# alitteneker/jsraytracer

Measured on AMD Instinct MI355X. Metric: pixel-samples/sec + %HBM-roofline, cornell_box_path 1024² @1/2/4/8 GPU, higher is better.
Workload: dtype f64; 1 GPU; cornell_box_path 1024x1024 64spp depth 8 (Incremental); width=1024, height=1024, spp=64, max_depth=8, parallelism=tiles1, col_block=1, headline=True, gather=rgba8

## Files before the change

jsraytracer_amd/csrc/device_common.h:

```cpp
#pragma once
#include <hip/hip_runtime.h>
#include <stdint.h>

#include "device_scene.h"
#include "fdlibm.h"
#include "js_number.h"

#define JSRT_HD __host__ __device__ __forceinline__

namespace jsrt {

#define JS_PI 3.141592653589793
#define DINF __builtin_inf()

JSRT_HD bool is_nan(double x) { return x != x; }
JSRT_HD double js_max(double a, double b) {
    double r = a > b ? a : b;
    if (a == b) r = __builtin_bit_cast(double, __builtin_bit_cast(uint64_t, a) & __builtin_bit_cast(uint64_t, b));
    return a != a ? a : r;
}
JSRT_HD double js_min(double a, double b) {
    double r = a < b ? a : b;
    if (a == b) r = __builtin_bit_cast(double, __builtin_bit_cast(uint64_t, a) | __builtin_bit_cast(uint64_t, b));
    return a != a ? a : r;
// ... 819 lines not shown
    }
    return res;
}

struct Hit {
    double t;
    int prim;
    int ctx;
};

template <int PF, class PT>
__device__ __forceinline__ double prim_intersect_local(const DScene &S, const PT &P, F3 o, F3 d, double minD,
                                                       double maxD) {
    switch (P.gkind) {
    case JSRT_GEOM_PLANE: return plane_t(o, d);
    case JSRT_GEOM_SQUARE: {
        const double t = plane_t(o, d);
        const F3 p = ray_point(o, d, t);
        return (-0.5f <= p.x && p.x <= 0.5f && -0.5f <= p.y && p.y <= 0.5f) ? t : -DINF;
    }
    case JSRT_GEOM_CIRCLE: {
        const double t = plane_t(o, d);
        const F3 p = ray_point(o, d, t);
        return (dot3(p, p) <= 1) ? t : -DINF;
    }
    case JSRT_GEOM_SPHERE: return sphere_static(o, d, minD);
    case JSRT_GEOM_CYLINDER: {
        const double oz = o.z, dz = d.z;
        if (fabs(oz) > 1 && dz != 0) minD = js_max(minD, -(oz - js_sign(oz)) / dz);
        const double t = sphere_static(f3(o.x, o.y, o.z * 0.0f), f3(d.x, d.y, d.z * 0.0f), minD);
        return (fabs(oz + t * dz) <= 1) ? t : -DINF;
    }
    case JSRT_GEOM_AABB: return aabb_intersect(P.center, P.half, o, d, minD, maxD);
    case JSRT_GEOM_TRIANGLE:
        if (PF & PF_TRI) return tri_intersect(S.tris[P.gindex], o, d);
        return -DINF;
    case JSRT_GEOM_SDF:
        if (PF & PF_SDF) return sdf_intersect(S, P.gindex, o, d, minD, maxD);
        return -DINF;
    default: return -DINF;
    }
}

template <class T>
JSRT_HD float xf_row_point(const T *r, F3 o) {
    return (float)((((double)o.x * r[0] + (double)o.y * r[1]) + (double)o.z * r[2]) + r[3]);
}
template <class T>
JSRT_HD float xf_row_dir(const T *r, F3 d) {
    return (float)(((double)d.x * r[0] + (double)d.y * r[1]) + (double)d.z * r[2]);
}

template <class T>
JSRT_HD double planar_intersect(int k, const T *inv, F3 o, F3 d, double minD, double lim) {
    const float oz = xf_row_point(inv + 8, o), dz = xf_row_dir(inv + 8, d);
    const double t = (dz != 0.0f) ? -(double)oz / (double)dz : -(double)__builtin_inf();
    if (k == JSRT_GEOM_PLANE || !(t > minD && t < lim)) return t;
    const float ox = xf_row_point(inv, o), oy = xf_row_point(inv + 4, o);
    const float dx = xf_row_dir(inv, d), dy = xf_row_dir(inv + 4, d);
    const F3 p = ray_point(f3(ox, oy, oz), f3(dx, dy, dz), t);
    if (k == JSRT_GEOM_SQUARE)
        return (-0.5f <= p.x && p.x <= 0.5f && -0.5f <= p.y && p.y <= 0.5f) ? t : -(double)__builtin_inf();
    return (dot3(p, p) <= 1) ? t : -(double)__builtin_inf();
}

#ifdef JSRT_X_F32XF
template <class T>
__device__ __forceinline__ float xf_row_point_x(const T *r, F3 o) {
    return fmaf(o.x, (float)r[0], fmaf(o.y, (float)r[1], fmaf(o.z, (float)r[2], (float)r[3])));
}
template <class T>
__device__ __forceinline__ float xf_row_dir_x(const T *r, F3 d) {
    return fmaf(d.x, (float)r[0], fmaf(d.y, (float)r[1], d.z * (float)r[2]));
}
#define XROWP xf_row_point_x
#define XROWD xf_row_dir_x
#else
#define XROWP xf_row_point
#define XROWD xf_row_dir
#endif

template <class T>
JSRT_HD int planar_any_f32(int k, const T *inv, F3 o, F3 d, double minD, double maxD, double &t_out) {
    constexpr float EPS = 4.76837158203125e-7f, EPSP = 3.814697265625e-6f, TINY = 1e-30f;
    const float oz = XROWP(inv + 8, o), dz = XROWD(inv + 8, d);
    if (dz == 0.0f) return 0;
#ifdef __HIP_DEVICE_COMPILE__
    const float ta = -oz * __builtin_amdgcn_rcpf(dz);
#else
    const float ta = -oz * (1.0f / dz);
#endif
    const float f0 = (float)minD, f1 = (float)maxD;
    if (!__builtin_isfinite(ta) || !__builtin_isfinite(f0) || !(fabsf(dz) >= 1e-30f)) return -1;
    const bool inf1 = !__builtin_isfinite(f1) && f1 > 0;
    const float et = EPS * fabsf(ta) + TINY, e0 = EPS * fabsf(f0) + TINY, e1 = inf1 ? 0.0f : EPS * fabsf(f1) + TINY;
    if (ta + et < f0 - e0 || (!inf1 && ta - et > f1 + e1)) return 0;
    if (!(ta - et > f0 + e0 && (inf1 || ta + et < f1 - e1))) return -1;
    if (k == JSRT_GEOM_PLANE) {
        t_out = ta;
        return 1;
    }
    const float ox = XROWP(inv, o), oy = XROWP(inv + 4, o);
    const float dx = XROWD(inv, d), dy = XROWD(inv + 4, d);
    const double td = (double)ta;
    const float sx = (float)((double)dx * td), sy = (float)((double)dy * td);
    const float px = ox + sx, py = oy + sy;
    const float ex = EPSP * (fabsf(sx) + fabsf(ox)) + TINY, ey = EPSP * (fabsf(sy) + fabsf(oy)) + TINY;
    if (!__builtin_isfinite(px) || !__builtin_isfinite(py) || !__builtin_isfinite(ex) || !__builtin_isfinite(ey))
        return -1;
    if (k == JSRT_GEOM_SQUARE) {
        if (fabsf(px) - ex > 0.5f || fabsf(py) - ey > 0.5f) return 0;
        if (fabsf(px) + ex < 0.5f && fabsf(py) + ey < 0.5f) {
            t_out = ta;
            return 1;
        }
        return -1;
    }
    const float sz = (float)((double)dz * td), pz = oz + sz;
    const float ez = EPSP * (fabsf(sz) + fabsf(oz)) + TINY;
    const double r2 = dot3(f3(px, py, pz), f3(px, py, pz));
    const double m = 2.0 * ((double)fabsf(px) * ex + (double)fabsf(py) * ey + (double)fabsf(pz) * ez) +
                     ((double)ex * ex + (double)ey * ey + (double)ez * ez) + 1e-15;
    if (!__builtin_isfinite(r2)) return -1;
    if (r2 - m > 1.0) return 0;
    if (r2 + m < 1.0) {
        t_out = ta;
        return 1;
    }
    return -1;
}

JSRT_HD int sphere_any_f32(F3 o, F3 d, double minD, double maxD, double &t_out, bool *second = nullptr) {
    constexpr float EPS = 4.76837158203125e-7f, EPSS = 1.9073486328125e-6f, TINY = 1e-30f;
    const double a = dot3(d, d), b = dot3(d, o), c = dot3(o, o) - 1;
    const double big = b * b - a * c;
    if (big < 0 || a == 0) return 0;
    if (!(big >= 1e-30) || !(a >= 1e-30) || !(a <= 1e30) || !(fabs(b) <= 1e30) || !(big <= 1e30)) return -1;
    const float fa = (float)a, fb = (float)b;
#ifdef __HIP_DEVICE_COMPILE__
    const float sq = __builtin_amdgcn_sqrtf((float)big), ia = __builtin_amdgcn_rcpf(fa);
#else
    const float sq = sqrtf((float)big), ia = 1.0f / fa;
#endif
    const float t1 = (-fb + sq) * ia, t2 = (-fb - sq) * ia;
    const float base = EPSS * (sq * ia);
    const float e1 = base + EPSS * fabsf(t1) + TINY, e2 = base + EPSS * fabsf(t2) + TINY;
    const float f0 = (float)minD, f1 = (float)maxD;
    if (!__builtin_isfinite(f0)) return -1;
    const bool inf1 = !__builtin_isfinite(f1) && f1 > 0;
    const float em = EPS * fabsf(f0) + TINY, eM = inf1 ? 0.0f : EPS * fabsf(f1) + TINY;
    float t, et;
    if (t2 - e2 > f0 + em) {
        t = t2;
        et = e2;
        if (second) *second = true;
// ... 17 lines not shown
    bool second = false;
    const int dec = sphere_any_f32(o, d, minD, lim, te, &second);
    if (dec != 1) return dec;
    const double a = dot3(d, d), b = dot3(d, o), c = dot3(o, o) - 1;
    const double big = sqrt(b * b - a * c);
    t_out = second ? (-b - big) / a : (-b + big) / a;
    return 1;
}

template <int PF, class PT>
__device__ __forceinline__ double prim_intersect(const DScene &S, const PT &P, F3 o, F3 d, double minD, double maxD,
                                                 bool transp, double lim) {
    if (!transp && !P.casts_shadow) return DINF;
    const int k = P.gkind;
    if (k == JSRT_GEOM_PLANE || k == JSRT_GEOM_SQUARE || k == JSRT_GEOM_CIRCLE) return planar_intersect(k, P.inv, o, d, minD, lim);
    return prim_intersect_local<PF>(S, P, xf_point(P.inv, o), xf_dir(P.inv, d), minD, maxD);
}

template <int PF, class PT>
__device__ __forceinline__ double prim_any(const DScene &S, const PT &P, F3 o, F3 d, double minD, double maxD,
                                           bool transp) {
#ifndef JSRT_NO_ANY_FILTER
    if (!transp && !P.casts_shadow) return DINF;
    const int k = P.gkind;
    double t = 0;
    if (k == JSRT_GEOM_AABB) {
#ifdef JSRT_X_F32XF
        const F3 lo = f3(XROWP(P.inv, o), XROWP(P.inv + 4, o), XROWP(P.inv + 8, o)),
                 ld = f3(XROWD(P.inv, d), XROWD(P.inv + 4, d), XROWD(P.inv + 8, d));
#else
        const F3 lo = xf_point(P.inv, o), ld = xf_dir(P.inv, d);
#endif
        const int dec = box_any_f32(P.center, P.half, lo, box_ray(ld), minD, maxD, t);
        if (dec >= 0) return dec ? t : -DINF;
        return aabb_intersect(P.center, P.half, lo, ld, minD, maxD);
    }
    if (k == JSRT_GEOM_PLANE || k == JSRT_GEOM_SQUARE || k == JSRT_GEOM_CIRCLE) {
        const int dec = planar_any_f32(k, P.inv, o, d, minD, maxD, t);
        if (dec >= 0) return dec ? t : -DINF;
        return planar_intersect(k, P.inv, o, d, minD, maxD);
    }
    if ((PF & PF_TRI) && k == JSRT_GEOM_TRIANGLE)
        return tri_any(S.tris[P.gindex], xf_point(P.inv, o), xf_dir(P.inv, d), minD, maxD);
    if (k == JSRT_GEOM_SPHERE) {
        const F3 lo = xf_point(P.inv, o), ld = xf_dir(P.inv, d);
        const int dec = sphere_any_f32(lo, ld, minD, maxD, t);
        if (dec >= 0) return dec ? t : -DINF;
        return sphere_static(lo, ld, minD);
    }
#endif
    return prim_intersect<PF>(S, P, o, d, minD, maxD, transp, maxD);
}

template <int PF, class PT>
__device__ __forceinline__ double prim_closest(const DScene &S, const PT &P, F3 o, F3 d, double minD, double maxD,
                                               bool transp, double lim) {
#if !defined(JSRT_NO_ANY_FILTER) && !defined(JSRT_NO_CLOSEST_FILTER)
    if constexpr (!(PF & PF_BVH)) {
        if (!transp && !P.casts_shadow) return DINF;
        const int k = P.gkind;
        double t = 0;
        if (k == JSRT_GEOM_AABB) {
            const F3 lo = xf_point(P.inv, o), ld = xf_dir(P.inv, d);
            const int dec = box_closest_f32(P.center, P.half, lo, ld, box_ray(ld), minD, lim, t);
            if (dec >= 0) return dec ? t : -DINF;
            return aabb_intersect(P.center, P.half, lo, ld, minD, maxD);
        }
        if (k == JSRT_GEOM_SPHERE) {
            const F3 lo = xf_point(P.inv, o), ld = xf_dir(P.inv, d);
            const int dec = sphere_closest_f32(lo, ld, minD, lim, t);
            if (dec >= 0) return dec ? t : -DINF;
            return sphere_static(lo, ld, minD);
        }
    }
#endif
    return prim_intersect<PF>(S, P, o, d, minD, maxD, transp, lim);
}

template <int PF, bool ANY>
__device__ __forceinline__ Hit bvh_cast(const DScene &S, const DInst &I, F3 o, F3 d, double minD, double maxD, bool transp) {
    Hit best{DINF, -1, I.ctx};
    const bool fast = I.count != 0;
    extern __shared__ int bvh_lds_stack[];
    int *const stack = bvh_lds_stack + threadIdx.x;
    const int stride = (int)blockDim.x;
    const BoxRay br = box_ray(d);
    const float fmin_d = (float)minD;
    float flim = (float)maxD;
    int sp = 0;
    stack[0] = I.first;
    ++sp;
    while (sp > 0) {
        --sp;
        const DBvhNode N = S.bvh[stack[sp * stride]];
#ifndef JSRT_NO_BOX_FILTER
        int en = box_enter_f32(N.cx, N.cy, N.cz, N.hx, N.hy, N.hz, o, br, fmin_d, flim);
#else
        int en = -1;
#endif
        if (en < 0) {
            double tmn, tmx;
            en = aabb_slab(N.cx, N.cy, N.cz, N.hx, N.hy, N.hz, o, d, minD, maxD, tmn, tmx) && tmn <= maxD &&
                 tmx >= minD && tmn <= best.t;
        }
        if (en) {
            if (N.b < 0) {
// ... 14 lines not shown
            } else {
                stack[sp * stride] = N.a;
                stack[(sp + 1) * stride] = N.b;
                sp += 2;
            }
        }
    }
    return best;
}

template <int PF, bool ANY>
__device__ __forceinline__ void nested_cast(const DScene &S, int inst, F3 o, F3 d, double minD, double maxD, bool transp, Hit &best) {
    struct Fr {
        int inst, next;
        F3 o, d;
    };
    Fr st[8];
    int sp = 0;
    {
        const DInst &I = S.insts[inst];
        st[sp++] = Fr{inst, 0, xf_point(S.mats + 12 * I.matrix, o), xf_dir(S.mats + 12 * I.matrix, d)};
    }
    while (sp > 0) {
        Fr &f = st[sp - 1];
        const DInst &I = S.insts[f.inst];
        if (I.kind == INST_BVH) {
            const Hit h = bvh_cast<PF, ANY>(S, I, f.o, f.d, minD, maxD, transp);
            --sp;
            if (h.prim >= 0 && h.t > minD && h.t < best.t && h.t < maxD) {
                best = h;
                if (ANY) return;
            }
            continue;
        }
        if (f.next >= I.count) { --sp; continue; }
        const int c = S.inst_child[I.first + f.next++];
        const DInst &C = S.insts[c];
        if (C.kind == INST_PRIM) {
            const double t = ANY ? prim_any<PF>(S, S.prims[C.prim], f.o, f.d, minD, maxD, transp)
                                 : prim_intersect<PF>(S, S.prims[C.prim], f.o, f.d, minD, maxD, transp, fmin(maxD, best.t));
            if (t > minD && t < best.t && t < maxD) {
                best = Hit{t, C.prim, I.ctx};
                if (ANY) return;
            }
        } else if (sp < 8) {
            const double *m = S.mats + 12 * C.matrix;
            const F3 no = xf_point(m, f.o), nd = xf_dir(m, f.d);
            st[sp++] = Fr{c, 0, no, nd};
        }
    }
}

template <class RBT>
__device__ __forceinline__ bool root_needed(const RBT &RB, F3 o, float ix, float iy, float iz, float oabs,
                                            float fminD, float flim) {
    if (!RB.bounded) return true;
    const float e = RB.k * oabs + RB.e0;
    float a0 = (RB.lo[0] - e - o.x) * ix, a1 = (RB.hi[0] + e - o.x) * ix;
    float tn = fminf(a0, a1), tf = fmaxf(a0, a1);
    a0 = (RB.lo[1] - e - o.y) * iy;
    a1 = (RB.hi[1] + e - o.y) * iy;
    tn = fmaxf(tn, fminf(a0, a1));
    tf = fminf(tf, fmaxf(a0, a1));
    a0 = (RB.lo[2] - e - o.z) * iz;
    a1 = (RB.hi[2] + e - o.z) * iz;
    tn = fmaxf(tn, fminf(a0, a1));
    tf = fminf(tf, fmaxf(a0, a1));
    return (tn <= tf) && (tf >= fminD) && (tn <= flim);
}

template <int PF, bool ANY>
__device__ __forceinline__ Hit world_cast(const DScene &S, F3 o, F3 d, double minD, double maxD, bool transp,
                                          uint64_t mask = ~0ull) {
    Hit best{DINF, -1, 0};
    const float ix = __builtin_amdgcn_rcpf(d.x), iy = __builtin_amdgcn_rcpf(d.y), iz = __builtin_amdgcn_rcpf(d.z);
    const float oabs = fmaxf(fabsf(o.x), fmaxf(fabsf(o.y), fabsf(o.z)));
    const float fminD = (float)minD;
    bool live = true;
    float flim = (float)maxD;
    for (int i = 0; i < S.n_roots; ++i) {
        if (i < 64 && !((mask >> i) & 1ull)) continue;
        const auto &R = as_const(S.rootrec)[i];
        const bool need = live && root_needed(R.rb, o, ix, iy, iz, oabs, fminD, flim);
        if (!__any(need)) continue;
#ifdef JSRT_X_CULLONLY
        if (ANY) continue;
#endif
        if (!need) {
        } else if (R.kind == INST_PRIM) {
            if (transp || R.p.casts_shadow) {
                const double t = ANY ? prim_any<PF>(S, R.p, o, d, minD, maxD, transp)
                                     : prim_closest<PF>(S, R.p, o, d, minD, maxD, transp, fmin(maxD, best.t));
                if (t > minD && t < best.t && t < maxD) {
                    best = Hit{t, R.prim, 0};
                    flim = (float)best.t;
                    if (ANY) live = false;
                }
            }
        } else if ((PF & PF_BVH) && R.kind == INST_BVH) {
            const auto *m = R.p.inv;
            const Hit h = bvh_cast<PF, ANY>(S, S.insts[R.inst], xf_point(m, o), xf_dir(m, d), minD, maxD, transp);
            if (h.prim >= 0 && h.t > minD && h.t < best.t && h.t < maxD) {
                best = h;
                flim = (float)best.t;
                if (ANY) live = false;
            }
        } else if (PF & PF_AGG) {
            nested_cast<PF, ANY>(S, R.inst, o, d, minD, maxD, transp, best);
            flim = (float)(best.t < maxD ? best.t : maxD);
            if (ANY && best.prim >= 0) live = false;
        }
    }
    return best;
}

template <int C>
__device__ __forceinline__ bool sroot_class(const DScene &S, uint64_t m, F3 o, F3 d, double minD, double maxD,
                                            float ix, float iy, float iz, float oabs, bool &live) {
    typedef uint32_t u16v __attribute__((ext_vector_type(16)));
    typedef uint32_t u8v __attribute__((ext_vector_type(8)));
    const float fminD = (float)minD, flim = (float)maxD;
    while (m) {
        if (!__any(live)) break;
        const int j = __builtin_ctzll(m);
        m &= m - 1;
        const CONST_AS uint32_t *w = reinterpret_cast<const CONST_AS uint32_t *>(as_const(S.sroot) + j);
        u16v a = *reinterpret_cast<const CONST_AS u16v *>(w);
        u16v b = *reinterpret_cast<const CONST_AS u16v *>(w + 16);
        u8v c = *reinterpret_cast<const CONST_AS u8v *>(w + 32);
        __asm__ volatile("" : "+s"(a), "+s"(b), "+s"(c));
        double inv[12];
#pragma unroll
        for (int k = 0; k < 8; ++k) inv[k] = __hiloint2double((int)a[2 * k + 1], (int)a[2 * k]);
#pragma unroll
        for (int k = 0; k < 4; ++k) inv[8 + k] = __hiloint2double((int)b[2 * k + 1], (int)b[2 * k]);
        RootBound rb;
        rb.lo[0] = __uint_as_float(b[8]);
        rb.lo[1] = __uint_as_float(b[9]);
        rb.lo[2] = __uint_as_float(b[10]);
        rb.k = __uint_as_float(b[11]);
        rb.hi[0] = __uint_as_float(b[12]);
        rb.hi[1] = __uint_as_float(b[13]);
        rb.hi[2] = __uint_as_float(b[14]);
        rb.e0 = __uint_as_float(b[15]);
        rb.bounded = (int32_t)c[7];
        const bool need = live && root_needed(rb, o, ix, iy, iz, oabs, fminD, flim);
        if (!__any(need)) continue;
        if (!need) continue;
        double t = 0;
        if constexpr (C == SR_BOX) {
            const float ce[3] = {__uint_as_float(c[0]), __uint_as_float(c[1]), __uint_as_float(c[2])};
            const float ha[3] = {__uint_as_float(c[4]), __uint_as_float(c[5]), __uint_as_float(c[6])};
            const F3 lo = xf_point(inv, o), ld = xf_dir(inv, d);
            const int dec = box_any_f32(ce, ha, lo, box_ray(ld), minD, maxD, t);
            if (dec < 0) t = aabb_intersect(ce, ha, lo, ld, minD, maxD);
            else if (!dec) t = -DINF;
        } else if constexpr (C == SR_PLANE || C == SR_SQUARE || C == SR_CIRCLE) {
            const int k = C == SR_PLANE ? JSRT_GEOM_PLANE : C == SR_SQUARE ? JSRT_GEOM_SQUARE : JSRT_GEOM_CIRCLE;
            const int dec = planar_any_f32(k, inv, o, d, minD, maxD, t);
            if (dec < 0) t = planar_intersect(k, inv, o, d, minD, maxD);
            else if (!dec) t = -DINF;
        } else if constexpr (C == SR_SPHERE) {
            const F3 lo = xf_point(inv, o), ld = xf_dir(inv, d);
            const int dec = sphere_any_f32(lo, ld, minD, maxD, t);
            if (dec < 0) t = sphere_static(lo, ld, minD);
            else if (!dec) t = -DINF;
// ... 338 lines not shown
```

jsraytracer_amd/csrc/render.hip:

```cpp
#include "render_levels.h"

#include <mutex>

namespace jsrt {

const char *const KT_NAMES[KT_N] = {"k_gen", "k_extend", "k_shade", "k_shadow", "k_reduce", "k_accum", "k_final",
                                    "k_resolve"};

__global__ __launch_bounds__(256) void k_gen(DScene S, RenderArgs A, WArgs W) {
    const uint32_t q = blockIdx.x * 256 + threadIdx.x;
    if ((!W.chain || W.hybrid) && q < LVL_UNDER) W.lvl[q] = q == 0 ? W.npaths : 0u;
    if (q >= W.npaths) return;
    int c = 0, py = 0, px = 0;
    const uint32_t nsb = W.npaths / W.npix;
    const uint32_t pl = W.pixel_major ? q / nsb : q % W.npix, sl = W.pixel_major ? q % nsb : q / W.npix;
    const uint32_t smp = W.s0 + sl;
    const bool valid = pixel_of(A, W.p0 + pl, c, py, px);
    if (!W.chain) {
        if (A.max_depth <= 0) {
            W.root[3 * q] = W.root[3 * q + 1] = W.root[3 * q + 2] = 0.0f;
            return;
        }
        W.path[q] = q;
        W.parent[q] = valid ? NO_PARENT : DEAD_RAY;
// ... 546 lines not shown
            release_events();
            return e;
        }
    }
    hipStream_t st2 = dual ? wf.side : st;
    const char *se = getenv("JSRT_SPLIT");
    const bool split = !timed_launches && ns > 0 && (se ? se[0] == '1' : (persist && !dual));
    auto aux_of = [&](Wavefront &w) -> hipError_t {
        hipError_t r = hipSuccess;
        if (!w.aux) r = hipStreamCreateWithFlags(&w.aux, hipStreamNonBlocking);
        if (r == hipSuccess && !w.ev_shade) r = hipEventCreateWithFlags(&w.ev_shade, hipEventDisableTiming);
        if (r == hipSuccess && !w.ev_shadow) r = hipEventCreateWithFlags(&w.ev_shadow, hipEventDisableTiming);
        return r;
    };
    if (split && (e = aux_of(wf)) == hipSuccess && dual) e = aux_of(*wf.twin);
    if (e != hipSuccess) {
        if (h_lvl) (void)hipHostFree(h_lvl);
        release_events();
        return e;
    }
    bool conservative = false, aborted = false;
    double reported = 0;
    for (int attempt = 0; e == hipSuccess; ++attempt) {
        if (kt) kt->attempts = (uint32_t)attempt + 1;
        const size_t cap = hybrid ? ((paths + paths * wf.pool_factor / 4 + 255) & ~(size_t)255) : paths;
        if (hybrid && cap * (size_t)depth >= ((size_t)1 << 32)) { e = hipErrorOutOfMemory; break; }
        const size_t pool = chain ? cap : paths * wf.pool_factor, level_cap = chain ? cap : pool / 2;
        int group = 1;
        const char *ss = getenv("JSRT_SHADOW_SERIAL");
        if (ns > 1 && ns <= 64 && !(ss && ss[0] == '1' && !persist))
            while (group < ns) group *= 2;
        const size_t hands = chain ? cap : std::max(level_cap, paths);
        const size_t shadow = persist ? hands * (size_t)group : 0;
        auto reserve = [&](Wavefront &w) {
            return chain ? w.reserve(cap, cap * (size_t)depth, cap, paths, sched, shadow)
                         : w.reserve(pool, pool, hands, paths, SCHED_TREE, shadow);
        };
        e = reserve(wf);
        if (e == hipSuccess && dual) {
            const hipError_t e2 = reserve(*wf.twin);
            if (e2 == hipErrorOutOfMemory) {
                (void)hipGetLastError();
                wf.twin->release();
                dual = false;
                st2 = st;
            } else {
                e = e2;
            }
        }
        if (e != hipSuccess) break;
        WArgs W = wf.args;
        W.ns = ns;
        W.group = group;
        W.chain = chain ? 1 : 0;
        W.hybrid = hybrid ? 1 : 0;
        W.cap = (uint32_t)cap;
        const char *be = getenv("JSRT_BUCKET");
        int shift = 0;
        while (S.n_prims > 0 && ((S.n_prims - 1) >> shift) >= BKT_N) ++shift;
        W.bucket = (learned && !persist && S.n_prims > 0 && ns > 0 && ns <= 64 && !(be && be[0] == '0')) ? shift + 1 : 0;
        W.pool = pool;
        W.level_cap = level_cap;
        const char *cs = getenv("JSRT_CHILD_SORT");
        W.child_sort = !chain && (cs ? (cs[0] == '1') : ((S.profile & PF_BVH) != 0));
        const char *bg = getenv("JSRT_BUCKET_GRID");
        const bool grid = bg ? bg[0] == '1' : S.profile == PF_ANALYTIC;
        W.bucket_grid = (W.bucket && S.grid_cells > 0 && grid) ? 1 : 0;
        W.pixel_major = pixel_major ? 1 : 0;
        WArgs W2 = W;
        if (dual) {
            const WArgs &t = wf.twin->args;
            W2.ox = t.ox; W2.oy = t.oy; W2.oz = t.oz; W2.dx = t.dx; W2.dy = t.dy; W2.dz = t.dz;
            W2.addr = t.addr; W2.key = t.key; W2.path = t.path; W2.parent = t.parent; W2.t = t.t;
            W2.prim = t.prim; W2.ctx = t.ctx; W2.node = t.node; W2.child = t.child; W2.slot = t.slot;
            W2.hand = t.hand; W2.hnode = t.hnode; W2.root = t.root; W2.lvl = t.lvl; W2.qctr = t.qctr; W2.sray = t.sray;
            W2.scol = t.scol; W2.bkt = t.bkt; W2.bbase = t.bbase; W2.brank = t.brank;
            W2.list0 = t.list0; W2.list1 = t.list1; W2.endl = t.endl;
            W2.fixrec = t.fixrec; W2.fixctr = t.fixctr; W2.fixcap = t.fixcap;
        }
        if ((e = hipMemsetAsync(A.accum, 0, (size_t)A.ncols * A.H * 4 * sizeof(float), st)) != hipSuccess) break;
        if ((e = hipMemsetAsync(W.lvl + LVL_UNDER, 0, 2 * sizeof(uint32_t), st)) != hipSuccess) break;
        if ((e = hipMemsetAsync(W.fixctr, 0, sizeof(uint32_t), st)) != hipSuccess) break;
        if (dual && (e = hipMemsetAsync(W2.fixctr, 0, sizeof(uint32_t), st)) != hipSuccess) break;
        if (dual) {
            if ((e = hipEventRecord(ev_start, st)) != hipSuccess || (e = hipStreamWaitEvent(st2, ev_start, 0)) != hipSuccess) break;
            if ((e = hipMemsetAsync(W2.lvl + LVL_UNDER, 0, 2 * sizeof(uint32_t), st2)) != hipSuccess) break;
        }
        auto read_flags = [&]() -> hipError_t {
            hipError_t r;
            if (dual && ((r = hipEventRecord(ev_end, st2)) != hipSuccess || (r = hipStreamWaitEvent(st, ev_end, 0)) != hipSuccess))
                return r;
            if ((r = hipMemcpyAsync(h_lvl, W.lvl, 64 * sizeof(uint32_t), hipMemcpyDeviceToHost, st)) != hipSuccess) return r;
            if (dual && (r = hipMemcpyAsync(h_lvl + 64, W2.lvl, 64 * sizeof(uint32_t), hipMemcpyDeviceToHost, st)) != hipSuccess)
                return r;
            return hipStreamSynchronize(st);
        };
        auto flagged = [&](int k) { return h_lvl[k] != 0 || (dual && h_lvl[64 + k] != 0); };
        uint64_t bi = 0;
        auto bounds = [&](uint32_t np) {
            std::vector<size_t> b(depth, 0);
            if (hybrid) {
                for (int L = 0; L < A.max_depth; ++L) {
                    b[L] = L == 0 ? np : cap;
                    if (L > 0 && !conservative && L < (int)wf.frac.size())
                        b[L] = std::min(cap, std::max<size_t>(256, (size_t)((double)np * wf.frac[L] * margin) + slack));
                }
// ... 141 lines not shown
```

jsraytracer_amd/csrc/render_kernel.h:

```cpp
#pragma once
#include <hip/hip_runtime.h>
#include <stdint.h>

#include <functional>
#include <vector>

#include "device_scene.h"

namespace jsrt {

constexpr int MAX_TREE_DEPTH = 16;
constexpr int LVL_FLAG = 63;
constexpr int LVL_UNDER = 62;
static_assert(2 * MAX_TREE_DEPTH + 2 <= LVL_UNDER, "hybrid chain count pairs lvl[2L, 2L + 1] below the flags");
constexpr int BKT_N = 64;
constexpr int BKT_S = 16;
constexpr int BKT_K = BKT_N * BKT_S;
constexpr int BKT_LEVEL = 3 * BKT_K + 64;

struct RenderArgs {
    int32_t W, H, kind, max_depth;
    int32_t s_begin, s_end, spp;
    uint32_t seed;
    int32_t x_offset, x_delt, col_block, ncols;
    float *accum;
    uint32_t *rgba;
    float *colors;
    int32_t final_pass;
    int32_t patches_x;
    int32_t patches;
    int32_t samples_per_batch;
    int32_t tile_p;
};

constexpr uint32_t INFO_HIT = 1u, INFO_LIT = 2u, INFO_MISS = 16u;
constexpr uint32_t INFO_UNIT0 = 32u, INFO_UNIT1 = 64u;
constexpr int INFO_NCHILD_SHIFT = 2;

struct WArgs {
    float *ox, *oy, *oz, *dx, *dy, *dz;
    uint32_t *addr;
    uint32_t *key;
    uint32_t *path;
    uint32_t *parent;
    double *t;
    int32_t *prim, *ctx;
    float4 *node;
    float4 *child;
    float4 *slot;
    float4 *hand;
    uint32_t *hnode;
    float *root;
    uint32_t *lvl;
    uint32_t *list0, *list1;
    uint8_t *endl;
    uint32_t *qctr;
    uint4 *fixrec;
    uint32_t *fixctr;
    uint32_t fixcap;
    int32_t force_fix;
    float4 *sray;
    float4 *scol;
    uint32_t *bkt;
    uint32_t *bbase;
    uint32_t *brank;
    uint32_t p0, npix, s0, npaths;
    int32_t ns;
    int32_t group;
    int32_t chain;
    int32_t hybrid;
    uint32_t cap;
    int32_t bucket;
    int32_t child_sort;
    int32_t bucket_grid;
    int32_t pixel_major;
    size_t pool, level_cap;
    size_t nstride, hstride;
    size_t sstride;
};

struct BatchSync {
    hipEvent_t wait = nullptr, done = nullptr;
    hipStream_t aux = nullptr;
    hipEvent_t shade_done = nullptr, shadow_done = nullptr;
};

struct Wavefront {
    void *mem = nullptr;
    Wavefront *twin = nullptr;
    hipStream_t side = nullptr;
    hipStream_t aux = nullptr;
    hipEvent_t ev_shade = nullptr, ev_shadow = nullptr;
    size_t pool_paths = 0, pool_factor = 8;
    int pool_mode = -1;
    bool fix_all = false;
    std::vector<double> frac;
    size_t cap_bytes = 0;
    WArgs args{};
    hipError_t reserve(size_t rays, size_t nodes, size_t hands, size_t paths, int mode, size_t shadow = 0);
    void release();
    ~Wavefront();
};

enum { KT_GEN, KT_EXTEND, KT_SHADE, KT_SHADOW, KT_REDUCE, KT_ACCUM, KT_FINAL, KT_RESOLVE, KT_N };
constexpr int SCHED_CHAIN = 0, SCHED_TREE = 1, SCHED_HYBRID = 2;
extern const char *const KT_NAMES[KT_N];

struct EventPairs {
    std::vector<hipEvent_t> b, e;
    size_t used = 0;
    void begin(hipStream_t s);
    void end(hipStream_t s);
    double total_ms(uint32_t *lost = nullptr) const;
    ~EventPairs();
};

struct KernelTimes {
    EventPairs ev[KT_N];
    uint32_t mask = ~0u;
    bool one_stream = false;
    uint32_t batches = 0;
// ... 31 lines not shown
```

jsraytracer_amd/csrc/render_levels.h:

```cpp
#pragma once
#include <hip/hip_runtime.h>
#include <stdint.h>
#include <stdlib.h>
#include <string.h>

#include <algorithm>
#include <vector>

#include "device_common.h"
#include "render_kernel.h"

#ifndef JSRT_SHADE_OCC
#define JSRT_SHADE_OCC 4
#endif
#ifndef JSRT_SHADE_OCC_SDF
#define JSRT_SHADE_OCC_SDF 3
#endif
#ifndef JSRT_SHADE_OCC_FLAT
#define JSRT_SHADE_OCC_FLAT 5
#endif
#ifndef JSRT_SHADOW_OCC
#define JSRT_SHADOW_OCC 6
#endif
#ifndef JSRT_SHADOW_OCC_FLAT
// ... 989 lines not shown
        if (shadow_cast_flat(S, P, delta, 0.0001, 1, mask)) return f3(0, 0, 0);
        return c;
    }
    const Hit sh = world_cast<PF, true>(S, P, delta, 0.0001, 1, false, mask);
    if (shadowed(sh)) return f3(0, 0, 0);
    return c;
}

__device__ __forceinline__ F3 light_sums(const DScene &S, uint32_t G, F3 ret, F3 c) {
    const int lane0 = (int)(__lane_id() & ~(G - 1));
    uint32_t k = 0;
    for (int li = 0; li < S.n_lights; ++li) {
        const DLight &Lt = S.lights[li];
        const int n = Lt.kind == JSRT_LIGHT_POINT ? 1 : Lt.samples;
        F3 light_color = f3(0, 0, 0);
        for (int j = 0; j < n; ++j, ++k) {
            const int src = lane0 + (int)k;
            light_color = add(light_color, f3(__shfl(c.x, src), __shfl(c.y, src), __shfl(c.z, src)));
        }
        if (n > 0) ret = add(ret, scale(light_color, Lt.inv_n));
    }
    return ret;
}

template <int PF, bool CHAIN, bool SERIAL, bool SPH, bool STAGE = false, bool FLAT = false>
__global__ __launch_bounds__(256, PF == PF_ANALYTIC ? JSRT_SHADOW_OCC_FLAT : JSRT_SHADOW_OCC) SHADOW_ATTR void k_shadow(
    DScene S, WArgs W, int L) {
    const LevelRange R = CHAIN ? chain_level(W, L) : level_range(W, L);
    const uint32_t count = R.count, base = R.base;
    const uint32_t G = (uint32_t)W.group, ns = (uint32_t)W.ns;
    const uint32_t e = blockIdx.x * 256 + threadIdx.x;
    uint32_t q = e / G;
    const uint32_t s = e % G;
    bool in = q < count;
    const float4 *hp = W.hand + (in ? q : 0u);
    uint32_t mi = 0;
    if (W.bucket) {
        in = q < as_const(W.bkt + (size_t)L * BKT_LEVEL)[3 * BKT_K];
        const uint32_t h = in ? q : 0u;
        q = W.hnode[h];
        mi = f2u(hp[W.hstride].w) & 0xFFu;
    }
    uint64_t mask = ~0ull;
    if (FLAT) mask = S.n_sroot >= 64 ? ~0ull : ((1ull << S.n_sroot) - 1);
    if (W.bucket && W.bucket_grid && S.grid_masked) {
        const uint64_t on = __ballot(in);
        if (on) {
            const uint32_t m0 = (uint32_t)__builtin_amdgcn_readlane((int)mi, __builtin_ctzll(on));
            if (!__ballot(in && mi != m0) && m0 <= (uint32_t)S.grid_cells)
                mask = FLAT ? as_const(S.grid_smask)[m0] : as_const(S.grid_mask)[m0];
        }
    }
    if (CHAIN && !W.bucket && in) q = chain_slot(W, L, q);
    const uint32_t i = base + (in ? q : 0u);
    const float4 nd = W.node[i];
    const bool lit = in && (f2u(nd.w) & INFO_LIT);
    F3 ret = f3(nd.x, nd.y, nd.z);
    if (SERIAL) {
        if (!lit) return;
        uint32_t k = 0;
        for (int li = 0; li < S.n_lights; ++li) {
            const DLight &Lt = S.lights[li];
            const int n = Lt.kind == JSRT_LIGHT_POINT ? 1 : Lt.samples;
            F3 light_color = f3(0, 0, 0);
            for (int j = 0; j < n; ++j, ++k)
                light_color = add(light_color, sample_color<PF, SPH>(S, hp[0], hp[W.hstride], hp, W.hstride, k, mask));
            if (n > 0) ret = add(ret, scale(light_color, Lt.inv_n));
        }
        W.node[i] = make_float4(ret.x, ret.y, ret.z, nd.w);
        return;
    }
    F3 c = f3(0, 0, 0);
    const float4 h0 = hp[0], h1 = hp[W.hstride];
    if constexpr (STAGE) {
        extern __shared__ uint4 stab_lds[];
        const uint4 *src = reinterpret_cast<const uint4 *>(S.stab);
        for (int k = (int)threadIdx.x; k < S.stab_words_shadow; k += 256) stab_lds[k] = src[k];
        __syncthreads();
        DScene SL = S;
        stab_bind(SL, stab_lds, false);
        if (lit && s < ns) c = sample_color<PF, SPH, FLAT>(SL, h0, h1, hp, W.hstride, s, mask);
    } else {
        if (lit && s < ns) c = sample_color<PF, SPH>(S, h0, h1, hp, W.hstride, s, mask);
    }
    ret = light_sums(S, G, ret, c);
    if (lit && s == 0) W.node[i] = make_float4(ret.x, ret.y, ret.z, nd.w);
}

struct ExtendSrc {
    const WArgs &W;
    uint32_t base;
    int L;
    __device__ __forceinline__ uint32_t ray(uint32_t j) const { return L >= 0 ? chain_slot(W, L, j) : base + j; }
    __device__ __forceinline__ bool load(uint32_t j, F3 &o, F3 &d) const {
        const uint32_t i = ray(j);
        if (W.prim[i] == NO_RAY) return false;
        o = f3(W.ox[i], W.oy[i], W.oz[i]);
        d = f3(W.dx[i], W.dy[i], W.dz[i]);
        return true;
    }
    __device__ __forceinline__ void store(uint32_t j, const Hit &h) const {
        const uint32_t i = ray(j);
        W.t[i] = h.t;
        W.prim[i] = h.prim;
        W.ctx[i] = h.ctx;
    }
};

template <int PF, bool CHAIN, bool FO>
__global__ __launch_bounds__(256, JSRT_MARCH_OCC) void k_extend_q(DScene S, WArgs W, int L, double minD) {
    const LevelRange R = CHAIN ? chain_level(W, L) : level_range(W, L);
    const uint32_t count = R.count, base = CHAIN ? 0u : R.base;
    ExtendSrc src{W, base, CHAIN ? L : -1};
    persistent_cast<PF, false, FO>(S, W.qctr + L, count, minD, DINF, true, src);
}

struct ShadowSrc {
    const WArgs &W;
    __device__ __forceinline__ bool load(uint32_t e, F3 &o, F3 &d) const {
        const float4 c = W.scol[e];
        if (f2u(c.w) != 1u) return false;
        const float4 a = W.sray[e], b = W.sray[W.sstride + e];
        o = f3(a.x, a.y, a.z);
        d = f3(b.x, b.y, b.z);
        return true;
    }
    __device__ __forceinline__ void store(uint32_t e, const Hit &h) const {
        if (shadowed(h)) W.scol[e].w = u2f(2u);
    }
};

template <int PF, bool CHAIN>
__global__ __launch_bounds__(256) void k_shadow_prep(DScene S, WArgs W, int L) {
    const LevelRange R = CHAIN ? chain_level(W, L) : level_range(W, L);
    const uint32_t count = R.count, base = R.base;
    const uint32_t G = (uint32_t)W.group, ns = (uint32_t)W.ns;
    const uint32_t e = blockIdx.x * 256 + threadIdx.x;
    const uint32_t q = e / G, s = e % G;
    if (q >= count || s >= ns) return;
// ... 105 lines not shown
        if (ev) kt->ev[which].end(s);
    };
    const size_t lds = (PF & (PF_BVH | PF_AGG)) ? bvh_lds_bytes(S, 256) : 0;
    const bool Q = (PF & PF_SDF) && W.sstride != 0;
    if (Q) (void)hipMemsetAsync(W.qctr, 0, 64 * sizeof(uint32_t), st);
    if (W.bucket) (void)hipMemsetAsync(W.bkt, 0, (size_t)MAX_TREE_DEPTH * BKT_LEVEL * sizeof(uint32_t), st);
    timed(KT_GEN, [&] { hipLaunchKernelGGL(k_gen, dim3(grid(W.npaths)), dim3(256), 0, st, S, A, W); });
    std::vector<size_t> ubs;
    const bool learned = !CHAIN || W.hybrid;
    for (int L = 0; L < A.max_depth && (!learned || bound[L] > 0); ++L) {
        const size_t ub = learned ? bound[L] : (size_t)W.npaths;
        ubs.push_back(ub);
        const int child_depth = A.max_depth - L - 1;
        timed(KT_EXTEND, [&] {
            if (Q && S.sdf_all_forms)
                hipLaunchKernelGGL((k_extend_q<PF, CHAIN, true>), dim3(persistent_grid((const void *)k_extend_q<PF, CHAIN, true>, ub)),
                                   dim3(256), 0, st, S, W, L, L == 0 ? 0.0 : 0.0001);
            else if (Q)
                hipLaunchKernelGGL((k_extend_q<PF, CHAIN, false>), dim3(persistent_grid((const void *)k_extend_q<PF, CHAIN, false>, ub)),
                                   dim3(256), 0, st, S, W, L, L == 0 ? 0.0 : 0.0001);
            else
                hipLaunchKernelGGL((k_extend<PF, CHAIN>), dim3(grid_ub(ub)), dim3(256), lds, st, S, W, L, L == 0 ? 0.0 : 0.0001);
        });
        if (W.bucket) hipLaunchKernelGGL(k_bucket_offsets, dim3(1), dim3(256), 0, st, W, L);
        if (split && L > 0 && W.ns > 0) (void)hipStreamWaitEvent(st, sync->shadow_done, 0);
        timed(KT_SHADE, [&] {
            if (PF == PF_ANALYTIC && S.stab_words > 0)
                hipLaunchKernelGGL((k_shade<PF, CHAIN, PF == PF_ANALYTIC>), dim3(grid_ub(ub)), dim3(256), (size_t)S.stab_words * 16,
                                   st, S, W, L, child_depth);
            else
                hipLaunchKernelGGL((k_shade<PF, CHAIN, false>), dim3(grid_ub(ub)), dim3(256), 0, st, S, W, L, child_depth);
            if (child_depth > 0) hipLaunchKernelGGL(k_fix_dirs, dim3(1), dim3(256), 0, st, W);
        });
        if (W.ns > 0 && split) {
            (void)hipEventRecord(sync->shade_done, st);
            (void)hipStreamWaitEvent(ss, sync->shade_done, 0);
        }
        if (W.ns > 0)
            timed(KT_SHADOW, [&] {
                const hipStream_t st = ss;
                const size_t ne = ub * (size_t)W.group;
                if (Q && W.ns <= 64) {
                    hipLaunchKernelGGL((k_shadow_prep<PF, CHAIN>), dim3(grid_ub(ne)), dim3(256), 0, st, S, W, L);
                    if (S.sdf_all_forms)
                        hipLaunchKernelGGL((k_shadow_cast<PF, CHAIN, true>),
                                           dim3(persistent_grid((const void *)k_shadow_cast<PF, CHAIN, true>, ne)), dim3(256), 0, st, S, W, L);
                    else
                        hipLaunchKernelGGL((k_shadow_cast<PF, CHAIN, false>),
                                           dim3(persistent_grid((const void *)k_shadow_cast<PF, CHAIN, false>, ne)), dim3(256), 0, st, S, W, L);
                    hipLaunchKernelGGL((k_shadow_sum<CHAIN>), dim3(grid_ub(ne)), dim3(256), 0, st, S, W, L);
                } else if (W.ns <= 1 || W.group > 1) {
                    const dim3 g(grid_ub(ub * (size_t)W.group));
                    const size_t sl = (size_t)S.stab_words_shadow * 16;
                    if (PF == PF_ANALYTIC && sl && S.sphere_lights && S.n_sroot > 0)
                        hipLaunchKernelGGL((k_shadow<PF, CHAIN, false, true, PF == PF_ANALYTIC, PF == PF_ANALYTIC>), g, dim3(256), sl, st, S, W, L);
                    else if (PF == PF_ANALYTIC && sl && S.n_sroot > 0)
                        hipLaunchKernelGGL((k_shadow<PF, CHAIN, false, false, PF == PF_ANALYTIC, PF == PF_ANALYTIC>), g, dim3(256), sl, st, S, W, L);
                    else if (PF == PF_ANALYTIC && sl && S.sphere_lights)
                        hipLaunchKernelGGL((k_shadow<PF, CHAIN, false, true, PF == PF_ANALYTIC>), g, dim3(256), sl, st, S, W, L);
                    else if (PF == PF_ANALYTIC && sl)
                        hipLaunchKernelGGL((k_shadow<PF, CHAIN, false, false, PF == PF_ANALYTIC>), g, dim3(256), sl, st, S, W, L);
                    else if (S.sphere_lights)
                        hipLaunchKernelGGL((k_shadow<PF, CHAIN, false, true>), g, dim3(256), lds, st, S, W, L);
                    else
                        hipLaunchKernelGGL((k_shadow<PF, CHAIN, false, false>), g, dim3(256), lds, st, S, W, L);
                } else if (S.sphere_lights) {
                    hipLaunchKernelGGL((k_shadow<PF, CHAIN, true, true>), dim3(grid_ub(ub)), dim3(256), lds, st, S, W, L);
                } else {
                    hipLaunchKernelGGL((k_shadow<PF, CHAIN, true, false>), dim3(grid_ub(ub)), dim3(256), lds, st, S, W, L);
                }
            });
        if (W.ns > 0 && split) (void)hipEventRecord(sync->shadow_done, ss);
    }
    if (split && W.ns > 0 && !ubs.empty()) (void)hipStreamWaitEvent(st, sync->shadow_done, 0);
    if (CHAIN && W.hybrid) {
        timed(KT_RESOLVE, [&] {
            for (int s = (int)ubs.size() - 1; s >= 1; --s)
                hipLaunchKernelGGL(k_resolve_side, dim3(grid_ub(ubs[s])), dim3(256), 0, st, A, W, s);
            hipLaunchKernelGGL(k_resolve_paths, dim3(grid(W.npaths)), dim3(256), 0, st, A, W);
        });
        accum_wait();
        timed(KT_ACCUM, [&] { hipLaunchKernelGGL(k_accum, dim3(grid(W.npix)), dim3(256), 0, st, A, W); });
        accum_done();
        return;
    }
    if (CHAIN) {
        accum_wait();
        timed(KT_RESOLVE, [&] { hipLaunchKernelGGL(k_resolve, dim3(grid(W.npix)), dim3(256), 0, st, A, W); });
        accum_done();
        return;
    }
    for (int L = (int)ubs.size() - 1; L >= 0; --L)
        timed(KT_REDUCE, [&] { hipLaunchKernelGGL(k_reduce, dim3(grid_ub(ubs[L])), dim3(256), 0, st, W, L); });
    accum_wait();
    timed(KT_ACCUM, [&] { hipLaunchKernelGGL(k_accum, dim3(grid(W.npix)), dim3(256), 0, st, A, W); });
    accum_done();
}

}
```

Before: 649.0 million pixel-samples/s.

## Add per-node shadow kernel tracing several light samples per thread

Adds a k_shadow_node kernel that traces up to four shadow samples per hit node in one thread. Each root's local-origin transform and slab bounds are computed once and shared across the samples, and the node accumulation is written once. This replaces the one-thread-per-sample k_shadow path for analytic scenes with a single non-sphere light when bucketing is on, and it is on by default through JSRT_SHADOW_NODE. It also changes the bucketed shade path to skip loading node data for lanes other than s == 0. The trade-off is fewer threads and more registers per thread, with wave-level __any loops that may diverge.

```diff
diff --git a/jsraytracer_amd/csrc/device_common.h b/jsraytracer_amd/csrc/device_common.h
--- a/jsraytracer_amd/csrc/device_common.h
+++ b/jsraytracer_amd/csrc/device_common.h
@@ -895,11 +895,11 @@
 }
 
 template <class T>
-JSRT_HD double planar_intersect(int k, const T *inv, F3 o, F3 d, double minD, double lim) {
-    const float oz = xf_row_point(inv + 8, o), dz = xf_row_dir(inv + 8, d);
+JSRT_HD double planar_intersect(int k, const T *inv, F3 o, F3 d, double minD, double lim, const F3 *lo = nullptr) {
+    const float oz = lo ? lo->z : xf_row_point(inv + 8, o), dz = xf_row_dir(inv + 8, d);
     const double t = (dz != 0.0f) ? -(double)oz / (double)dz : -(double)__builtin_inf();
     if (k == JSRT_GEOM_PLANE || !(t > minD && t < lim)) return t;
-    const float ox = xf_row_point(inv, o), oy = xf_row_point(inv + 4, o);
+    const float ox = lo ? lo->x : xf_row_point(inv, o), oy = lo ? lo->y : xf_row_point(inv + 4, o);
     const float dx = xf_row_dir(inv, d), dy = xf_row_dir(inv + 4, d);
     const F3 p = ray_point(f3(ox, oy, oz), f3(dx, dy, dz), t);
     if (k == JSRT_GEOM_SQUARE)
@@ -924,9 +924,10 @@
 #endif
 
 template <class T>
-JSRT_HD int planar_any_f32(int k, const T *inv, F3 o, F3 d, double minD, double maxD, double &t_out) {
+JSRT_HD int planar_any_f32(int k, const T *inv, F3 o, F3 d, double minD, double maxD, double &t_out,
+                           const F3 *lo = nullptr) {
     constexpr float EPS = 4.76837158203125e-7f, EPSP = 3.814697265625e-6f, TINY = 1e-30f;
-    const float oz = XROWP(inv + 8, o), dz = XROWD(inv + 8, d);
+    const float oz = lo ? lo->z : XROWP(inv + 8, o), dz = XROWD(inv + 8, d);
     if (dz == 0.0f) return 0;
 #ifdef __HIP_DEVICE_COMPILE__
     const float ta = -oz * __builtin_amdgcn_rcpf(dz);
@@ -943,7 +944,7 @@
         t_out = ta;
         return 1;
     }
-    const float ox = XROWP(inv, o), oy = XROWP(inv + 4, o);
+    const float ox = lo ? lo->x : XROWP(inv, o), oy = lo ? lo->y : XROWP(inv + 4, o);
     const float dx = XROWD(inv, d), dy = XROWD(inv + 4, d);
     const double td = (double)ta;
     const float sx = (float)((double)dx * td), sy = (float)((double)dy * td);
@@ -1067,6 +1068,45 @@
     return prim_intersect<PF>(S, P, o, d, minD, maxD, transp, maxD);
 }
 
+template <class PT>
+JSRT_HD F3 prim_local_origin(const PT &P, F3 o) { return xf_point(P.inv, o); }
+
+template <class PT>
+JSRT_HD bool prim_any_local(const PT &P, F3 o, F3 lo, F3 d, double minD, double maxD, double &out) {
+    const int k = P.gkind;
+    double t = 0;
+    out = 0;
+    if (k == JSRT_GEOM_AABB) {
+        const F3 ld = xf_dir(P.inv, d);
+        const int dec = box_any_f32(P.center, P.half, lo, box_ray(ld), minD, maxD, t);
+        out = dec >= 0 ? (dec ? t : -DINF) : aabb_intersect(P.center, P.half, lo, ld, minD, maxD);
+        return true;
+    }
+    if (k == JSRT_GEOM_PLANE || k == JSRT_GEOM_SQUARE || k == JSRT_GEOM_CIRCLE) {
+        const int dec = planar_any_f32(k, P.inv, o, d, minD, maxD, t, &lo);
+        out = dec >= 0 ? (dec ? t : -DINF) : planar_intersect(k, P.inv, o, d, minD, maxD, &lo);
+        return true;
+    }
+    if (k == JSRT_GEOM_SPHERE) {
+        const F3 ld = xf_dir(P.inv, d);
+        const int dec = sphere_any_f32(lo, ld, minD, maxD, t);
+        out = dec >= 0 ? (dec ? t : -DINF) : sphere_static(lo, ld, minD);
+        return true;
+    }
+    return false;
+}
+
+template <int PF, class PT>
+__device__ __forceinline__ double prim_any_at(const DScene &S, const PT &P, F3 o, F3 lo, F3 d, double minD,
+                                              double maxD, bool transp) {
+#ifndef JSRT_NO_ANY_FILTER
+    if (!transp && !P.casts_shadow) return DINF;
+    double t;
+    if (prim_any_local(P, o, lo, d, minD, maxD, t)) return t;
+#endif
+    return prim_any<PF>(S, P, o, d, minD, maxD, transp);
+}
+
 template <int PF, class PT>
 __device__ __forceinline__ double prim_closest(const DScene &S, const PT &P, F3 o, F3 d, double minD, double maxD,
                                                bool transp, double lim) {
@@ -1187,7 +1227,7 @@
 }
 
 template <class RBT>
-__device__ __forceinline__ bool root_needed(const RBT &RB, F3 o, float ix, float iy, float iz, float oabs,
+JSRT_HD bool root_needed(const RBT &RB, F3 o, float ix, float iy, float iz, float oabs,
                                             float fminD, float flim) {
     if (!RB.bounded) return true;
     const float e = RB.k * oabs + RB.e0;
@@ -1247,6 +1287,76 @@
         }
     }
     return best;
+}
+
+struct RootSlab {
+    float lx, hx, ly, hy, lz, hz;
+};
+template <class RBT>
+JSRT_HD RootSlab root_slab(const RBT &RB, F3 o, float oabs) {
+    const float e = RB.k * oabs + RB.e0;
+    return RootSlab{RB.lo[0] - e - o.x, RB.hi[0] + e - o.x, RB.lo[1] - e - o.y,
+                    RB.hi[1] + e - o.y, RB.lo[2] - e - o.z, RB.hi[2] + e - o.z};
+}
+JSRT_HD bool root_needed_at(const RootSlab &B, float ix, float iy, float iz, float fminD, float flim) {
+    float a0 = B.lx * ix, a1 = B.hx * ix;
+    float tn = fminf(a0, a1), tf = fmaxf(a0, a1);
+    a0 = B.ly * iy;
+    a1 = B.hy * iy;
+    tn = fmaxf(tn, fminf(a0, a1));
+    tf = fminf(tf, fmaxf(a0, a1));
+    a0 = B.lz * iz;
+    a1 = B.hz * iz;
+    tn = fmaxf(tn, fminf(a0, a1));
+    tf = fminf(tf, fmaxf(a0, a1));
+    return (tn <= tf) && (tf >= fminD) && (tn <= flim);
+}
+
+template <int PF, int NS>
+__device__ __forceinline__ uint32_t world_any_node(const DScene &S, F3 o, const F3 (&d)[NS], uint32_t live, double minD,
+                                                   double maxD, uint64_t mask) {
+    static_assert(!(PF & (PF_BVH | PF_AGG)), "flat scenes only");
+    float ix[NS], iy[NS], iz[NS];
+#pragma unroll
+    for (int s = 0; s < NS; ++s) {
+        ix[s] = __builtin_amdgcn_rcpf(d[s].x);
+        iy[s] = __builtin_amdgcn_rcpf(d[s].y);
+        iz[s] = __builtin_amdgcn_rcpf(d[s].z);
+    }
+    const float oabs = fmaxf(fabsf(o.x), fmaxf(fabsf(o.y), fabsf(o.z)));
+    const float fminD = (float)minD, flim = (float)maxD;
+    for (int i = 0; i < S.n_roots; ++i) {
+        if (i < 64 && !((mask >> i) & 1ull)) continue;
+        if (!__any(live != 0u)) break;
+        const auto &R = as_const(S.rootrec)[i];
+        uint32_t need = live;
+        if (R.rb.bounded) {
+            const RootSlab B = root_slab(R.rb, o, oabs);
+            need = 0u;
+#pragma unroll
+            for (int s = 0; s < NS; ++s)
+                if (((live >> s) & 1u) && root_needed_at(B, ix[s], iy[s], iz[s], fminD, flim)) need |= 1u << s;
+        }
+        if (!__any(need != 0u)) continue;
+        if (R.kind != INST_PRIM || !R.p.casts_shadow) continue;
+        if (need) {
+            const F3 lo = prim_local_origin(R.p, o);
+#pragma nounroll
+            for (int s = 0; s < NS; ++s) {
+                const bool mine = (need >> s) & 1u;
+                if (!__any(mine)) continue;
+                F3 ds = d[0];
+#pragma unroll
+                for (int k = 1; k < NS; ++k)
+                    if (s == k) ds = d[k];
+                if (mine) {
+                    const double t = prim_any_at<PF>(S, R.p, o, lo, ds, minD, maxD, false);
+                    if (t > minD && t < maxD) live &= ~(1u << s);
+                }
+            }
+        }
+    }
+    return live;
 }
 
 template <int C>
diff --git a/jsraytracer_amd/csrc/render.hip b/jsraytracer_amd/csrc/render.hip
--- a/jsraytracer_amd/csrc/render.hip
+++ b/jsraytracer_amd/csrc/render.hip
@@ -622,6 +622,8 @@
         WArgs W = wf.args;
         W.ns = ns;
         W.group = group;
+        const char *sn = getenv("JSRT_SHADOW_NODE");
+        W.shadow_node = (sn ? sn[0] == '1' : true) ? 1 : 0;
         W.chain = chain ? 1 : 0;
         W.hybrid = hybrid ? 1 : 0;
         W.cap = (uint32_t)cap;
diff --git a/jsraytracer_amd/csrc/render_kernel.h b/jsraytracer_amd/csrc/render_kernel.h
--- a/jsraytracer_amd/csrc/render_kernel.h
+++ b/jsraytracer_amd/csrc/render_kernel.h
@@ -67,6 +67,7 @@
     uint32_t p0, npix, s0, npaths;
     int32_t ns;
     int32_t group;
+    int32_t shadow_node;
     int32_t chain;
     int32_t hybrid;
     uint32_t cap;
diff --git a/jsraytracer_amd/csrc/render_levels.h b/jsraytracer_amd/csrc/render_levels.h
--- a/jsraytracer_amd/csrc/render_levels.h
+++ b/jsraytracer_amd/csrc/render_levels.h
@@ -1065,9 +1065,12 @@
         }
     }
     if (CHAIN && !W.bucket && in) q = chain_slot(W, L, q);
+    const bool slots_lit = PF != PF_ANALYTIC && W.bucket;
+    if (slots_lit) in = in && q < (CHAIN ? W.cap : count);
     const uint32_t i = base + (in ? q : 0u);
-    const float4 nd = W.node[i];
-    const bool lit = in && (f2u(nd.w) & INFO_LIT);
+    float4 nd = make_float4(0.0f, 0.0f, 0.0f, 0.0f);
+    if (!slots_lit || s == 0) nd = W.node[i];
+    const bool lit = in && (slots_lit || (f2u(nd.w) & INFO_LIT));
     F3 ret = f3(nd.x, nd.y, nd.z);
     if (SERIAL) {
         if (!lit) return;
@@ -1098,6 +1101,84 @@
     }
     ret = light_sums(S, G, ret, c);
     if (lit && s == 0) W.node[i] = make_float4(ret.x, ret.y, ret.z, nd.w);
+}
+
+#ifndef JSRT_SHADOW_NODE_OCC
+#define JSRT_SHADOW_NODE_OCC 5
+#endif
+template <int PF, bool CHAIN, int NS>
+__global__ __launch_bounds__(256, JSRT_SHADOW_NODE_OCC) void k_shadow_node(DScene S, WArgs W, int L) {
+    const LevelRange R = CHAIN ? chain_level(W, L) : level_range(W, L);
+    const uint32_t count = R.count, base = R.base;
+    const uint32_t ns = (uint32_t)W.ns;
+    const uint32_t e = blockIdx.x * 256 + threadIdx.x;
+    const bool in = e < as_const(W.bkt + (size_t)L * BKT_LEVEL)[3 * BKT_K];
+    const uint32_t h = in ? e : 0u;
+    const float4 *hp = W.hand + h;
+    const size_t hs = W.hstride;
+    const uint32_t q = W.hnode[h];
+    const float4 h0 = hp[0], h1 = hp[hs];
+    const uint32_t tag = f2u(h1.w);
+    uint64_t mask = ~0ull;
+    if (W.bucket_grid && S.grid_masked) {
+        const uint32_t mi = tag & 0xFFu;
+        const uint64_t on = __ballot(in);
+        if (on) {
+            const uint32_t m0 = (uint32_t)__builtin_amdgcn_readlane((int)mi, __builtin_ctzll(on));
+            if (!__ballot(in && mi != m0) && m0 <= (uint32_t)S.grid_cells) mask = as_const(S.grid_mask)[m0];
+        }
+    }
+    const bool lit = in && q < (CHAIN ? W.cap : count);
+    const uint32_t i = base + (lit ? q : 0u);
+    const float4 nd = W.node[i];
+    extern __shared__ uint4 stab_lds[];
+    const uint4 *src = reinterpret_cast<const uint4 *>(S.stab);
+    for (int k = (int)threadIdx.x; k < S.stab_words_shadow; k += 256) stab_lds[k] = src[k];
+    __syncthreads();
+    if (!lit) return;
+    DScene SL = S;
+    stab_bind(SL, stab_lds, false);
+    const F3 P = f3(h0.x, h0.y, h0.z);
+    const jsrt_rec_material &M = SL.mat[(tag & HAND_MAT) >> 8];
+    ShadeData sd;
+    sd.N = f3(h1.x, h1.y, h1.z);
+    sd.diff = (tag & HAND_DIFF) ? f3(hp[2 * hs].x, hp[2 * hs].y, hp[2 * hs].z) : mc_const3(SL, M.diffuse);
+    sd.spec = (tag & HAND_SPEC) ? f3(hp[4 * hs].x, hp[4 * hs].y, hp[4 * hs].z) : mc_const3(SL, M.specular);
+    sd.R = f3(0, 0, 0);
+    sd.refr = f3(0, 0, 0);
+    sd.kr = 1.0;
+    if (tag & HAND_R) {
+        const float4 h3 = hp[3 * hs];
+        sd.R = f3(h3.x, h3.y, h3.z);
+        if (tag & HAND_KR) {
+            const float4 h5 = hp[5 * hs];
+            sd.refr = f3(h5.x, h5.y, h5.z);
+            sd.kr = __hiloint2double((int)f2u(h3.w), (int)f2u(h5.w));
+        }
+    }
+    sd.smoothness = M.smoothness;
+    const int mkind = (int)M.kind;
+    F3 d[NS], c[NS];
+    uint32_t live = 0u;
+#pragma unroll
+    for (int s = 0; s < NS; ++s) {
+        d[s] = f3(1, 1, 1);
+        c[s] = f3(0, 0, 0);
+        if ((uint32_t)s < ns) {
+            RngH rng{f2u(h0.w), (uint32_t)SL.sample_call[s]};
+            F3 Ld, lcol;
+            light_sample<false>(SL, as_const(S.lights)[0], P, rng, d[s], Ld, lcol);
+            c[s] = light_sample_color(mkind, sd, Ld, lcol, !(tag & HAND_R));
+            if (!(c[s].x == 0.0f && c[s].y == 0.0f && c[s].z == 0.0f)) live |= 1u << s;
+        }
+    }
+    live = world_any_node<PF, NS>(S, P, d, live, 0.0001, 1, mask);
+    F3 light_color = f3(0, 0, 0);
+#pragma unroll
+    for (int s = 0; s < NS; ++s)
+        if ((uint32_t)s < ns) light_color = add(light_color, ((live >> s) & 1u) ? c[s] : f3(0, 0, 0));
+    const F3 ret = add(f3(nd.x, nd.y, nd.z), scale(light_color, as_const(S.lights)[0].inv_n));
+    W.node[i] = make_float4(ret.x, ret.y, ret.z, nd.w);
 }
 
 struct ExtendSrc {
@@ -1309,7 +1390,14 @@
                 } else if (W.ns <= 1 || W.group > 1) {
                     const dim3 g(grid_ub(ub * (size_t)W.group));
                     const size_t sl = (size_t)S.stab_words_shadow * 16;
-                    if (PF == PF_ANALYTIC && sl && S.sphere_lights && S.n_sroot > 0)
+                    bool node_form = false;
+                    if constexpr (PF == PF_ANALYTIC)
+                        node_form = W.shadow_node && W.bucket && sl && S.n_lights == 1 && !S.sphere_lights && S.n_sroot == 0 &&
+                                    W.ns > 1 && W.ns <= 4;
+                    if (node_form) {
+                        if constexpr (PF == PF_ANALYTIC)
+                            hipLaunchKernelGGL((k_shadow_node<PF, CHAIN, 4>), dim3(grid_ub(ub)), dim3(256), sl, st, S, W, L);
+                    } else if (PF == PF_ANALYTIC && sl && S.sphere_lights && S.n_sroot > 0)
                         hipLaunchKernelGGL((k_shadow<PF, CHAIN, false, true, PF == PF_ANALYTIC, PF == PF_ANALYTIC>), g, dim3(256), sl, st, S, W, L);
                     else if (PF == PF_ANALYTIC && sl && S.n_sroot > 0)
                         hipLaunchKernelGGL((k_shadow<PF, CHAIN, false, false, PF == PF_ANALYTIC, PF == PF_ANALYTIC>), g, dim3(256), sl, st, S, W, L);
```

Result: faster. 682.4 million pixel-samples/s (median of 6 runs) (+5.1%).
